# marius311/MuseInference.jl

Hardware: AMD Instinct MI355X
Metric: MC sims/sec (MAP+score) (higher is better)
Workload: dtype f64; 1 GPU; funnel_1e4: Neal's funnel family model=funnel, N=10000-dim z, 1-dim theta, nsims=512 per step (512 on this rank), cold start z0=0, atol=1e-2; element_split=1, parallelism=sims sharded over 1 GPU(s) (weak scaling), one all-gather of scores per step

## Files before the change

museinference.jl_amd/csrc/kernels.hpp:

```cpp
#pragma once
#include <hip/hip_runtime.h>
#include <math.h>
#include <hip/hip_ext.h>
#include <stdint.h>
#include <type_traits>
#include "../../include/muse_hip.h"
#include "solver.hpp"
#include "step.hpp"

namespace muse {



typedef __attribute__((address_space(4))) const uint32_t* kernarg_ptr;
template <bool RAW>
__device__ __forceinline__ void load_problem_theta(const BatchArgs& a, double* args_lds, int p, int tid) {
    if (a.nmaps > 1) {
        wg_barrier<RAW>();
        asm volatile("" : "+v"(tid));
        if (tid < (int)(sizeof(MapTheta) / 4)) {
            uint32_t* dst = reinterpret_cast<uint32_t*>(args_lds) + offsetof(BatchArgs, cur) / 4;
            kernarg_ptr kp = (kernarg_ptr)__builtin_amdgcn_kernarg_segment_ptr();
            dst[tid] = kp[(offsetof(BatchArgs, maps) + (size_t)(p / a.n_per_map) * sizeof(MapTheta)) / 4 + tid];
        }
        wg_barrier<RAW>();
    }
}

template <class P>
struct JacobiPlace : P {};
template <class P>
struct place_is_jacobi : std::false_type {};
template <class P>
struct place_is_jacobi<JacobiPlace<P>> : std::true_type {};

template <class Model, class Place, bool IMPLICIT = false>
__global__ void __launch_bounds__(Place::T) __attribute__((amdgpu_waves_per_eu(Place::kWavesPerEu)))
map_score_kernel(const BatchArgs ) {
    constexpr bool JACOBI = place_is_jacobi<Place>::value;
    static_assert(!JACOBI || (IMPLICIT && !Model::kStencil), "the preconditioned loop is the implicit branch's, for the elementwise models");
    extern __shared__ __attribute__((aligned(16))) unsigned char smem[];
    constexpr int T = Place::T;
    double* red = reinterpret_cast<double*>(smem);
    double* shs = red + 2 * (T / 64) * 8;
    int* ticket = reinterpret_cast<int*>(shs + 40);
    double* args_lds = shs + 42;
    const int tid = threadIdx.x;
#ifdef MUSE_STAMPS
    unsigned long long t_entry;
    asm volatile("s_memtime %0\n\ts_waitcnt lgkmcnt(0)" : "=s"(t_entry)::"memory");
#endif
    {
        kernarg_ptr kp = (kernarg_ptr)__builtin_amdgcn_kernarg_segment_ptr();
        uint32_t* dst = reinterpret_cast<uint32_t*>(args_lds);
        for (int w = tid; w < (int)(kArgsHeadBytes / 4); w += T) dst[w] = kp[w];
        if (tid == 0) ticket[2] = 0;
    }
    __syncthreads();
    const BatchArgs& a = *reinterpret_cast<const BatchArgs*>(args_lds);
    double* exch = args_lds + kArgsDoubles;
    double* lds_x = exch + (Place::kCluster ? kMaxCluster * 8 : 0);
    double* lds_g = lds_x + a.ld + 2;
    const bool wave0 = (__builtin_amdgcn_readfirstlane(tid) >> 6) == 0;
    auto clock_stamp = [&](int k) {
        if (a.clock_out && blockIdx.x == 0 && wave0) {
            unsigned long long t0, t1;
            asm volatile("s_memtime %0\n\ts_memrealtime %1\n\ts_waitcnt lgkmcnt(0)" : "=s"(t0), "=s"(t1)::"memory");
            a.clock_out[2 * k] = t0;
            a.clock_out[2 * k + 1] = t1;
        }
    };
    clock_stamp(0);
    if constexpr (Place::kXgLds) {
        if (tid == 0) {
            lds_x[a.ld] = 0.0;
            lds_g[a.ld] = 0.0;
            lds_x[a.ld + 1] = 0.0;
            lds_g[a.ld + 1] = 0.0;
            if (a.N < a.ld) {
                lds_x[a.N] = 0.0;
                lds_g[a.N] = 0.0;
            }
        }
    }
    if constexpr (Place::kCluster) {
        const int csize = a.csize;
        const int cluster = a.xcd_local ? ((int)(blockIdx.x >> 3) / csize) * 8 + (int)(blockIdx.x & 7) : (int)blockIdx.x / csize;
        const int crank = a.xcd_local ? (int)(blockIdx.x >> 3) % csize : (int)blockIdx.x % csize;
        double* cl_scratch = a.scratch + (int64_t)cluster * a.scratch_stride;
        Solver<Model, Place> sv(a, tid, red, shs);
        sv.crank = crank;
        sv.csize = csize;
        sv.tfirst = crank * T + tid;
        sv.pstride = csize * T;
        sv.pack_blocks();
        sv.cl_part = a.cl_part + (size_t)cluster * kClusterSlotDoubles;
        sv.exch = exch;
        sv.cl_epoch = a.cl_state[cluster];
        int nth = 0;
#ifdef MUSE_STAMPS
        if (tid == 0 && a.stamps && cluster < a.nproblems) a.stamps[(size_t)cluster * 16 + 8] = t_entry;
#endif
        for (int p = cluster; p < a.nproblems; p += a.nclusters, ++nth) {
            sv.bufsel = nth & 1;
            sv.next_p = p + a.nclusters < a.nproblems ? p + a.nclusters : -1;
            sv.parity = 0;
            wg_barrier<!Model::kStencil>();
            load_problem_theta<!Model::kStencil>(a, args_lds, p, tid);
            if constexpr (IMPLICIT && Model::kPair) sv.template run_implicit_pair<JACOBI>(p, cl_scratch, lds_x, lds_g);
            else if constexpr (IMPLICIT) sv.template run_implicit<JACOBI>(p, cl_scratch, lds_x, lds_g);
            else sv.run(p, cl_scratch, lds_x, lds_g);
        }
#ifdef MUSE_STAMPS
        if (cluster < a.nproblems) sv.stamp(cluster + ((a.nproblems - 1 - cluster) / a.nclusters) * a.nclusters, 9);
#endif
        clock_stamp(1);
        if (tid == 0 && crank == 0) {
            a.cl_state[cluster] = sv.cl_epoch;
            if (cluster == 0) a.error_flag[1] = (int)(sv.cl_epoch >> 1);
        }
    } else {
        double* wg_scratch = a.scratch + (int64_t)blockIdx.x * a.scratch_stride;
        unsigned pk0, pk1;
        {
            Solver<Model, Place> s0(a, tid, red, shs);
            s0.pack_blocks();
            pk0 = s0.pk[0];
            pk1 = s0.pk[1];
        }
        int p = (int)blockIdx.x;
        for (;;) {
            int next = 0;
            if (tid == 0) next = atomicAdd(a.work_counter, 1);
#ifdef MUSE_STAMPS
            if (tid == 0 && a.stamps && p < (int)gridDim.x) a.stamps[(size_t)p * 16 + 8] = t_entry;
#endif
            load_problem_theta<!Model::kStencil>(a, args_lds, p, tid);
            {
                Solver<Model, Place> sv(a, tid, red, shs);
                sv.pk[0] = pk0;
                sv.pk[1] = pk1;
                if constexpr (IMPLICIT && Model::kPair) sv.template run_implicit_pair<JACOBI>(p, wg_scratch, lds_x, lds_g);
                else if constexpr (IMPLICIT) sv.template run_implicit<JACOBI>(p, wg_scratch, lds_x, lds_g);
                else sv.run(p, wg_scratch, lds_x, lds_g);
            }
            wg_barrier<!Model::kStencil>();
            if (tid == 0) ticket[0] = next;
            wg_barrier<!Model::kStencil>();
            p = (int)gridDim.x + (__builtin_amdgcn_readfirstlane(ticket[0]) - a.ticket_base);
            if (p >= a.nproblems) break;
        }
        clock_stamp(1);
    }
}

constexpr int kLoopArgsDoubles = (int)((sizeof(LoopArgs) + 7) / 8);
constexpr int kLoopRecDoubles = 7 * kMaxTheta + kMaxTheta * kMaxTheta + 1;
constexpr int kLoopPersistDoubles = kLoopArgsDoubles + kLoopRecDoubles + 3;
enum { STEP_TIMEOUT = 100 };

template <class Place>
struct LoopLds {
    BatchArgs* a;
    double *red, *shs, *lds_x, *lds_g, *persist, *stepbuf, *rec;
    LoopArgs* L;
    int* flags;
    unsigned long long* t_prev;
    __device__ __forceinline__ LoopLds(unsigned char* smem) {
        unsigned z = 0;
        asm volatile("" : "+s"(z));
        red = reinterpret_cast<double*>(smem + z);
        shs = red + 2 * (Place::T / 64) * 8;
        double* args_lds = shs + 42;
        a = reinterpret_cast<BatchArgs*>(args_lds);
        lds_x = args_lds + kArgsDoubles;
        lds_g = lds_x + a->ld + 2;
        persist = Place::kXgLds ? lds_g + a->ld + 2 : lds_x;
        stepbuf = Place::kXgLds ? lds_x : persist + kLoopPersistDoubles;
        L = reinterpret_cast<LoopArgs*>(persist);
        rec = persist + kLoopArgsDoubles;
        flags = reinterpret_cast<int*>(rec + kLoopRecDoubles);
        t_prev = reinterpret_cast<unsigned long long*>(rec + kLoopRecDoubles + 2);
    }
};

#if defined(MUSE_USER_MODEL_HEADER) && defined(MUSE_MODEL_PAIR)
__device__ __forceinline__ void pair_theta_update(int lane, int nt, const int64_t* bnd, const double* th, MapTheta& m) {
    const int K = nt >> 1;
    if (lane < K) {
        double cf[4] = {0.0, 0.0, 0.0, 0.0};
        (void)muse_model_coefs(th[lane], th[K + lane], cf);
        m.t.theta[lane] = th[lane];
        m.t.theta[K + lane] = th[K + lane];
        double* rec = &m.t.sd[0] + 4 * lane;
        rec[0] = cf[0];
        rec[1] = cf[1];
        rec[2] = cf[2];
        rec[3] = cf[3];
    } else if (lane < kMaxTheta / 2) {
        double* rec = &m.t.sd[0] + 4 * lane;
        rec[0] = rec[1] = rec[2] = rec[3] = 0.0;
    }
    if (lane >= 2 * K && lane < kMaxTheta) m.t.theta[lane] = 0.0;
    if (lane == kMaxTheta) {
        double cst = 0.0;
        for (int k = 0; k < K; ++k) {
            double cf[4] = {0.0, 0.0, 0.0, 0.0};
            const double C = muse_model_coefs(th[k], th[K + k], cf);
            cst += (double)(bnd[k + 1] - bnd[k]) * C;
        }
        m.f_const = cst;
        m.pad_ = 0.0;
    }
}
#endif

template <class Model, class Place>
__global__ void __launch_bounds__(Place::T) __attribute__((amdgpu_waves_per_eu(Place::kWavesPerEu)))
muse_loop_kernel(const BatchArgs , const LoopArgs ) {
    static_assert(!Place::kCluster, "one workgroup per element");
    extern __shared__ __attribute__((aligned(16))) unsigned char smem[];
    constexpr int T = Place::T, NW = T / 64;
    const int tid = threadIdx.x;
    {
        kernarg_ptr kp = (kernarg_ptr)__builtin_amdgcn_kernarg_segment_ptr();
        uint32_t* dst = reinterpret_cast<uint32_t*>(reinterpret_cast<double*>(smem) + 2 * (T / 64) * 8 + 42);
        for (int w = tid; w < (int)(kArgsHeadBytes / 4); w += T) dst[w] = kp[w];
    }
    __syncthreads();
    {
        LoopLds<Place> m(smem);
        kernarg_ptr kp = (kernarg_ptr)__builtin_amdgcn_kernarg_segment_ptr();
        uint32_t* dst = reinterpret_cast<uint32_t*>(m.persist);
        for (int w = tid; w < (int)(sizeof(LoopArgs) / 4); w += T) dst[w] = kp[sizeof(BatchArgs) / 4 + w];
        if (tid == 0) {
            unsigned long long now;
            asm volatile("s_memrealtime %0\n\ts_waitcnt lgkmcnt(0)" : "=s"(now)::"memory");
            *m.t_prev = now;
            m.flags[0] = m.flags[1] = m.flags[2] = 0;
        }
    }
    unsigned pk0, pk1;
    {
        LoopLds<Place> m(smem);
        Solver<Model, Place> s0(*m.a, tid, m.red, m.shs);
        s0.pack_blocks();
        pk0 = s0.pk[0];
        pk1 = s0.pk[1];
    }
    const bool solving = ((kernarg_ptr)__builtin_amdgcn_kernarg_segment_ptr())[(sizeof(BatchArgs) + offsetof(LoopArgs, stepper_solves)) / 4] != 0;
    const int stepper_id = (int)gridDim.x - 1;
    const int nworkers = solving ? (int)gridDim.x : (int)gridDim.x - 1;
    const bool stepper = (int)blockIdx.x == stepper_id;
    Prefetch<Place::EPT> pf;
    pf.p = -1;
    pf.have_n1 = pf.have_n2 = pf.have_x = pf.have_xg = pf.g_pending = false;
    typename Place::VZ zkeep;
    zkeep.clear();
    typedef __attribute__((address_space(1))) unsigned long long gu64;
#ifdef MUSE_STAMPS
    auto loop_stamp = [&](int k) {
        LoopLds<Place> m(smem);
        const int b = (int)blockIdx.x, row = b == stepper_id ? 2 : (b == 0 ? 0 : (b == stepper_id / 2 ? 1 : -1));
        if (tid == 0 && m.a->stamps && row >= 0) {
            unsigned long long t;
            asm volatile("s_memrealtime %0\n\ts_waitcnt lgkmcnt(0)" : "=s"(t)::"memory");
            m.a->stamps[(size_t)(m.a->nproblems + row) * 16 + k] = t;
        }
    };
#else
    auto loop_stamp = [](int) {};
#endif
    auto iteration_setup = [&](int it) {
        LoopLds<Place> m(smem);
        BatchArgs& a = *m.a;
        const LoopArgs& L = *m.L;
        a.z0_mode = (it > 1 || L.z0_warm) ? Z0_WARM : Z0_ZERO;
        if (it > 1 && a.ncache) a.ncache_mode = 2;
        a.scores = L.scores_out + (int64_t)(it - 1) * L.scores_stride;
        a.info = L.info_out + (int64_t)(it - 1) * L.info_stride;
        a.gran_tag = L.tag_base + (unsigned)it;
        if constexpr (Place::kXgLds) {
            m.lds_x[a.ld] = 0.0;
            m.lds_g[a.ld] = 0.0;
            m.lds_x[a.ld + 1] = 0.0;
            m.lds_g[a.ld + 1] = 0.0;
            if (a.N < a.ld && pf.p < 0) {
                m.lds_x[a.N] = 0.0;
                m.lds_g[a.N] = 0.0;
            }
        }
    };
    if (!stepper) {
    for (int iter = 1;; ++iter) {
        int err = STEP_OK, converged = 0;
        if (iter == 1 && tid == 0) iteration_setup(1);
        __syncthreads();
        {
            loop_stamp(0);
            {
                LoopLds<Place> m(smem);
                const BatchArgs& a = *m.a;
// ... 603 lines not shown
```

museinference.jl_amd/csrc/muse_engine.cpp:

```cpp
#include <hip/hip_runtime.h>
#include <math.h>
#include <stdint.h>
#include <stdio.h>
#include <stdlib.h>
#include <string.h>

#include <chrono>
#include <string>
#include <thread>
#include <utility>
#include <vector>

#include "../../include/muse_hip.h"
#include "args.hpp"
#include "host_loop.h"
#include "switches.hpp"
#include "user_model.hpp"

using namespace muse;

#if defined(__x86_64__) || defined(__i386__)
#define MUSE_CPU_RELAX() __builtin_ia32_pause()
#elif defined(__aarch64__)
#define MUSE_CPU_RELAX() asm volatile("yield" ::: "memory")
// ... 188 lines not shown
    if (pl == P_R512x10) fixed += (size_t)2 * (c->ld + 2) * sizeof(double);
    return fixed;
}
static int64_t place_scratch_vectors(int pl) {
    return (pl == P_S256 || pl == P_S512) ? 4 + 2 * kM + 1 : pl == P_C256 ? 4 + 2 * kM + 1 + 2 : 2 * kM;
}

static int ensure_zhat(muse_ctx* c, int64_t slots) {
    if (slots <= c->lane->zhat_slots) return MUSE_OK;
    double* nz = nullptr;
    if (hipMalloc(&nz, (size_t)slots * c->ld * sizeof(double)) != hipSuccess)
        return fail(MUSE_ERR_ALLOC, "hipMalloc(zhat) failed");
    HIPCHK(hipMemsetAsync(nz, 0, (size_t)slots * c->ld * sizeof(double), c->lane->stream));
    if (c->lane->zhat) {
        HIPCHK(hipMemcpyAsync(nz, c->lane->zhat, (size_t)c->lane->zhat_slots * c->ld * sizeof(double), hipMemcpyDeviceToDevice,
                              c->lane->stream));
        HIPCHK(hipStreamSynchronize(c->lane->stream));
        HIPCHK(hipFree(c->lane->zhat));
    }
    c->lane->zhat = nz;
    c->lane->zhat_slots = slots;
    return MUSE_OK;
}
static int ensure_scratch(muse_ctx* c, size_t doubles) {
    if (doubles <= c->lane->scratch_doubles) return MUSE_OK;
    HIPCHK(hipStreamSynchronize(c->lane->stream));
    if (c->lane->scratch) HIPCHK(hipFree(c->lane->scratch));
    c->lane->scratch = nullptr;
    c->lane->scratch_doubles = 0;
    if (hipMalloc(&c->lane->scratch, doubles * sizeof(double)) != hipSuccess)
        return fail(MUSE_ERR_ALLOC, "hipMalloc(scratch) failed");
    c->lane->scratch_doubles = doubles;
    return MUSE_OK;
}
static bool ensure_ncache(muse_ctx* c, int64_t slots) {
    if (!ncache_applies(c)) return false;
    if (slots <= c->ncache_slots) return true;
    if (hipStreamSynchronize(c->lane->stream) != hipSuccess) return false;
    if (c->ncache) hipFree(c->ncache);
    c->ncache = nullptr;
    c->ncache_slots = 0;
    c->nc_count = 0;
    if (hipMalloc(&c->ncache, (size_t)slots * 2 * c->ld * sizeof(double)) != hipSuccess) {
        (void)hipGetLastError();
        static bool warned = false;
        if (!warned) {
            fprintf(stderr, "[libmuse_hip] normals cache of %lld slots not allocated: simulations are re-drawn by the generator\n",
                    (long long)slots);
            warned = true;
        }
        return false;
    }
    c->ncache_slots = slots;
    return true;
}
static size_t result_bytes(const muse_ctx* c, int64_t cap) {
    return (size_t)cap * (size_t)c->ntheta * sizeof(double) + (size_t)cap * sizeof(muse_info);
}
static bool ncache_holds(const muse_ctx* c, uint64_t seed, int64_t sim0, int64_t count) {
    return c->ncache && c->nc_count > 0 && c->nc_seed == seed && sim0 >= c->nc_sim0 && sim0 + count <= c->nc_sim0 + c->nc_count;
}
static int ensure_results(muse_ctx* c, int area, int64_t n) {
    if (n <= c->res_cap[area]) return MUSE_OK;
    HIPCHK(hipStreamSynchronize(c->lane->stream));
    if (c->scores_pin[area]) HIPCHK(hipHostFree(c->scores_pin[area]));
    const int64_t cap = n + n / 2 + 16;
    HIPCHK(hipHostMalloc(&c->scores_pin[area], result_bytes(c, cap), hipHostMallocDefault));
    c->info_pin[area] = reinterpret_cast<muse_info*>(c->scores_pin[area] + cap * c->ntheta);
    c->scores_dev[area] = c->scores_pin[area];
    c->info_dev[area] = c->info_pin[area];
    c->res_cap[area] = cap;
    return MUSE_OK;
}

static void common_args(const muse_ctx* c, BatchArgs& a, int64_t stamp_rows) {
    a.N = c->N;
    a.ld = c->ld;
    a.ntheta = c->ntheta;
    for (int k = 0; k <= kMaxTheta; ++k) {
        a.bnd[k] = c->bnd[k];
        a.bnd32[k] = k < nblocks_of(c->ntheta) ? (int)c->bnd[k] : 0x7fffffff;
    }
    a.x_data = c->x_data;
    if (!a.zhat) a.zhat = c->lane->zhat;
    a.work_counter = c->lane->counter;
    if (a.nmaps <= 1) {
        a.nmaps = 1;
        a.n_per_map = a.nproblems;
        a.map_stride = a.nproblems;
    }
    a.debug = c->debug & 0xffff;
    a.stamps = (c->stamps && stamp_rows <= c->stamps_cap) ? c->stamps : nullptr;
    a.csize = 1;
    a.error_flag = c->lane->error_flag;
}
static void attach_ncache(BatchArgs& a, double* cache, int64_t sim0, int64_t count, int mode) {
    a.ncache = cache;
    a.ncache_sim0 = sim0;
    a.ncache_count = (int)count;
    a.ncache_mode = mode;
}

static int launch_batch(muse_ctx* c, BatchArgs& a, hipEvent_t done = nullptr, bool jacobi = false) {
    common_args(c, a, a.nproblems);
    a.clock_out = c->prof_on ? c->clock_pin : nullptr;
    const bool implicit = a.kind == BATCH_IMPLICIT;
    const int pl = implicit ? (use_cluster(c) ? P_C256 : P_S512) : choose_place(c);
    int grid = c->num_cus * place_wgs_per_cu(pl);
    if (place_is_cluster(pl) && c->comm_reserve_cus > 0 && c->num_cus > 2 * c->comm_reserve_cus)
        grid = (c->num_cus - c->comm_reserve_cus) * place_wgs_per_cu(pl);
    if (place_is_cluster(pl) && c->nlanes > 1) grid /= c->nlanes;
    if (place_is_cluster(pl)) {
        const int sharers = c->sw.shared_gpu_ranks;
        if (sharers > 1) grid = grid / sharers > 0 ? grid / sharers : 1;
    }
    a.nclusters = 0;
    if (place_is_cluster(pl)) {
        a.csize = cluster_size(c);
        int ncl = grid / a.csize;
        if (ncl > a.nproblems) ncl = a.nproblems;
        if (ncl < 1) ncl = 1;
        a.nclusters = ncl;
        grid = ncl * a.csize;
        const bool wrap = c->lane->error_flag[1] > 0x30000000;
        if (ncl > c->lane->cl_cap || wrap) {
            HIPCHK(hipStreamSynchronize(c->lane->stream));
            const int cap = ncl > c->lane->cl_cap ? ncl : c->lane->cl_cap;
            if (c->lane->cl_part) HIPCHK(hipFree(c->lane->cl_part));
            if (c->lane->cl_state) HIPCHK(hipFree(c->lane->cl_state));
            c->lane->cl_part = nullptr; c->lane->cl_state = nullptr; c->lane->cl_cap = 0;
            HIPCHK(hipMalloc(&c->lane->cl_part, (size_t)cap * kClusterSlotDoubles * sizeof(double)));
            HIPCHK(hipMalloc(&c->lane->cl_state, (size_t)cap * sizeof(unsigned int)));
            HIPCHK(hipMemsetAsync(c->lane->cl_part, 0, (size_t)cap * kClusterSlotDoubles * sizeof(double), c->lane->stream));
            HIPCHK(hipMemsetAsync(c->lane->cl_state, 0, (size_t)cap * sizeof(unsigned int), c->lane->stream));
            c->lane->error_flag[1] = 0;
            c->lane->cl_cap = cap;
        }
        a.cl_part = c->lane->cl_part;
        a.cl_state = c->lane->cl_state;
        a.xcd_local = (!c->sw.no_xcd_local && ncl % 8 == 0 && !stencil_ctx(c)) ? 1 : 0;
    } else {
        if (grid > a.nproblems) grid = a.nproblems;
        if (grid < 1) grid = 1;
    }
    a.scratch_stride = place_scratch_vectors(pl) * c->ld;
    int rc = ensure_scratch(c, (size_t)(place_is_cluster(pl) ? a.nclusters : grid) * a.scratch_stride);
    if (rc) return rc;
    a.scratch = c->lane->scratch;
    const size_t lds = place_lds(c, pl);
    if (c->lane->ticket_base > 0x70000000u) {
        HIPCHK(hipMemsetAsync(c->lane->counter, 0, 16, c->lane->stream));
        c->lane->ticket_base = 0;
    }
    a.ticket_base = (int)c->lane->ticket_base;
    if (!place_is_cluster(pl)) c->lane->ticket_base += (unsigned)a.nproblems;
    hipEvent_t e0 = c->ev0, e1 = c->ev1;
    if (c->prof_on && (size_t)(2 * c->prof_count + 1) < c->prof_ev.size()) {
        e0 = c->prof_ev[2 * c->prof_count];
        e1 = c->prof_ev[2 * c->prof_count + 1];
        c->prof_count += 1;
    }
    const bool timed = c->timing || c->prof_on;
    if (timed) HIPCHK(hipEventRecord(e0, c->lane->stream));
    {
        LaunchShape shape;
        shape.model = c->model; shape.ntheta = c->ntheta; shape.place = pl; shape.grid = grid; shape.implicit = implicit; shape.lds = lds;
        shape.jacobi = implicit && jacobi;
        shape.big = tier_big(c, pl, a.nmaps);
        shape.lds_s = !implicit && pl == P_C256 && stencil_lds_s(c, a.csize);
        shape.taps = c->stencil_taps;
        shape.noise = c->noise_on;
        shape.link = c->link_on;
        shape.done_event = done;
        const hipError_t e = launch_solver(shape, a, c->lane->stream);
        if (e == hipErrorNotSupported && shape.jacobi)
            rc = fail(MUSE_ERR_INVALID, "this model's preconditioned implicit-differentiation kernel keeps more than 256 bytes of scratch per "
                                        "lane (a header too heavy for its registers): MUSE_IMPLICIT_PL_JACOBI is refused for this library "
                                        "rather than run slower than the loop it replaces -- call without the bit");
        else if (e != hipSuccess) rc = fail(MUSE_ERR_HIP, std::string("solver launch: ") + hipGetErrorString(e));
    }
    if (rc) return rc;
    if (timed) {
        HIPCHK(hipEventRecord(e1, c->lane->stream));
        c->last0 = e0;
        c->last1 = e1;
        c->ev_valid = true;
    }
    return MUSE_OK;
}

static int create_lane(muse_ctx* c, int l) {
    LaneState& ln = c->lanes[l];
    if (ln.ready) return MUSE_OK;
    if (l == 0) ln.stream = c->own_stream;
    else HIPCHK(hipStreamCreateWithFlags(&ln.stream, hipStreamNonBlocking));
    HIPCHK(hipMalloc(&ln.counter, 16));
    HIPCHK(hipMemset(ln.counter, 0, 16));
    HIPCHK(hipHostMalloc(&ln.error_flag, 64, hipHostMallocDefault));
    ln.error_flag[0] = ln.error_flag[1] = 0;
    ln.ready = true;
    return MUSE_OK;
}
static void free_lane(muse_ctx* c, int l) {
    LaneState& ln = c->lanes[l];
    if (!ln.ready) return;
    hipFree(ln.scratch); hipFree(ln.counter); hipFree(ln.cl_part); hipFree(ln.cl_state); hipHostFree(ln.error_flag);
    hipFree(ln.zhat);
    if (l != 0) hipStreamDestroy(ln.stream);
    ln = LaneState();
}
static int use_lane(muse_ctx* c, int l) {
    const int rc = create_lane(c, l);
    if (rc) return rc;
    c->lane = &c->lanes[l];
    return MUSE_OK;
}
template <class F>
static int for_each_lane(muse_ctx* c, F&& f) {
    int rc = MUSE_OK;
    for (int l = 0; l < kMaxLanes && rc == MUSE_OK; ++l)
        if (c->lanes[l].ready) rc = f(c->lanes[l]);
    return rc;
}
static int drain_lanes(muse_ctx* c) {
    return for_each_lane(c, [](LaneState& ln) -> int {
        HIPCHK(hipStreamSynchronize(ln.stream));
        return MUSE_OK;
    });
}

static int settle_area(muse_ctx* c, int area) {
    if (!c->area_inflight[area] || c->nlanes <= 1) return MUSE_OK;
    return drain_lanes(c);
}

#if defined(MUSE_USER_MODEL_HEADER) && defined(MUSE_MODEL_NCONST)
extern "C" {
const double* muse_host_consts[MUSE_MODEL_MAX_CONST] = {nullptr, nullptr, nullptr, nullptr};
long muse_host_const_len[MUSE_MODEL_MAX_CONST] = {0, 0, 0, 0};
}
static muse_ctx* g_consts_owner = nullptr;
static void own_host_constants(muse_ctx* c) {
    if (!c->has_consts || g_consts_owner == c) return;
    for (int k = 0; k < MUSE_MODEL_MAX_CONST; ++k) {
        muse_host_consts[k] = c->consts_host[k];
        muse_host_const_len[k] = c->consts_len[k];
    }
    g_consts_owner = c;
}
#define MUSE_OWN_CONSTANTS(c) own_host_constants(c)
#else
#define MUSE_OWN_CONSTANTS(c) do { } while (0)
#endif
static void set_launch_constants(const muse_ctx* c, BatchArgs& a) {
    for (int k = 0; k < 4; ++k) {
        a.consts[k] = c->consts_dev[k];
        a.const_len[k] = c->consts_len[k];
    }
    if (c->stencil_taps || c->noise_on || c->link_on)
        for (int k = 0; k < kStencilWeights; ++k) a.taps[k] = c->stencil_w[k];
    if (c->noise_on)
        for (int k = 0; k < 2; ++k) a.consts[k] = c->noise_dev[k];
    if (c->link_on) {
        for (int k = 0; k < 2; ++k) a.link[k] = c->link_a[k];
        if (!c->noise_on) a.consts[0] = a.consts[1] = c->link_unit;
    }
}

static int ensure_link_unit(muse_ctx* c, const char* who) {
    if (c->link_unit) return MUSE_OK;
    std::vector<double> ones((size_t)c->ld, 0.0);
    for (int64_t i = 0; i < c->N; ++i) ones[(size_t)i] = 1.0;
    double* fresh = nullptr;
    hipError_t e = hipMalloc(&fresh, (size_t)c->ld * sizeof(double));
    if (e == hipSuccess) e = hipMemcpy(fresh, ones.data(), (size_t)c->ld * sizeof(double), hipMemcpyHostToDevice);
    if (e != hipSuccess) {
        hipFree(fresh);
        return fail(MUSE_ERR_HIP, std::string(who) + ": the unit noise vector: " + hipGetErrorString(e));
    }
    c->link_unit = fresh;
    return MUSE_OK;
}

extern "C" {

const char* muse_last_error(void) { return g_err.c_str(); }
int64_t muse_max_resident_n(void) { return kMaxResidentN; }

const char* muse_model_name(int model) {
#ifdef MUSE_USER_MODEL_HEADER
    return model == MUSE_MODEL_USER ? MUSE_MODEL_NAME : nullptr;
#else
    static const char* const names[3] = {"funnel", "noise", "smooth"};
    return model >= 0 && model <= 2 ? names[model] : nullptr;
#endif
}

int muse_ctx_create(int model, int64_t N, int ntheta, int device, muse_ctx** out) {
    if (!out) return fail(MUSE_ERR_INVALID, "out is NULL");
    *out = nullptr;
    if (model < 0 || model > MUSE_MODEL_USER) return fail(MUSE_ERR_INVALID, "unknown model");
    if (!muse_model_name(model))
        return fail(MUSE_ERR_INVALID, model == MUSE_MODEL_USER
                                          ? "MUSE_MODEL_USER: this library holds the built-in models only (build one from a model "
                                            "header, include/muse_model.h)"
                                          : "this library was built from a user's model header and holds MUSE_MODEL_USER only");
    if (N < 1) return fail(MUSE_ERR_INVALID, "N must be >= 1");
// ... 1631 lines not shown
```

museinference.jl_amd/csrc/solver.hpp:

```cpp
#pragma once
#include <math.h>

#include "models.hpp"
#include "reduce.hpp"
#include "rng.hpp"

namespace muse {

template <int EPT>
struct Prefetch {
    int p;
    bool have_n1;
    bool have_n2;
    bool have_x;
    bool have_xg;
    bool g_pending;
};
#ifndef MUSE_NORMALS_AUX
#define MUSE_NORMALS_AUX 0
#endif
constexpr int kNormalsAux = MUSE_NORMALS_AUX;
typedef __attribute__((address_space(1))) const void* glds_src_t;
typedef __attribute__((address_space(3))) void* glds_dst_t;
template <int T, int EPT>
__device__ __forceinline__ void prefetch_issue(const BatchArgs& a, int tid, int p, double* lds_x, double* lds_g, Prefetch<EPT>& pf,
                                               bool both) {
    const ProblemDesc d = describe(a, p);
    const int64_t ld = a.ld;
    const bool sim = d.x_mode == X_SAMPLE && d.nslot >= 0;
    pf.p = p;
    pf.have_n1 = sim;
    pf.have_n2 = sim && both;
    pf.have_x = d.x_mode == X_DATA && both;
    pf.have_xg = d.x_mode == X_DATA && !both && !(a.debug & 256);
    pf.g_pending = (sim || pf.have_xg) && !both;
    int tl = tid;
    asm volatile("" : "+v"(tl));
    const double* src_x = sim ? a.ncache + (int64_t)(2 * d.nslot + 1) * ld : a.x_data;
    const double* src_g = pf.have_xg ? a.x_data : a.ncache + (int64_t)(2 * d.nslot) * ld;
    const int wave0 = __builtin_amdgcn_readfirstlane(tl) & ~63;
#pragma unroll
    for (int j = 0; j < EPT; ++j) {
        const int i0 = 2 * (tl + j * T);
        if (i0 < (int)ld) {
            const int base = 2 * (wave0 + j * T);
            if (pf.have_n2 || pf.have_x) __builtin_amdgcn_global_load_lds((glds_src_t)(src_x + i0), (glds_dst_t)(lds_x + base), 16, 0, kNormalsAux);
            if (pf.have_n1 || pf.have_xg) __builtin_amdgcn_global_load_lds((glds_src_t)(src_g + i0), (glds_dst_t)(lds_g + base), 16, 0, kNormalsAux);
        }
    }
}

template <bool PAIR>
struct PairState {};
template <>
struct PairState<true> {
    double pc[4], psd[2];
};
template <class Model, class Place>
constexpr bool uniform_linesearch() { return !(Place::kResident && Place::kXgLds && Model::MAXB > 1); }
template <class Model, class Place, bool UNIFORM_LS = uniform_linesearch<Model, Place>()>
struct Solver : PairState<Model::kPair> {
    static constexpr int T = Place::T, EPT = Place::EPT, U = Place::U, MAXB = Model::MAXB;
    static constexpr bool kBig = MAXB > kMaxTheta;
    static constexpr int KB = kBig ? 1 : MAXB;
    static_assert(!kBig || !Place::kResident, "the big tier runs in the streaming placements");
    const double* big_sd;
    const double* big_iv;
    double big_rcpN;
    const BatchArgs& a;
    const int tid;
    double* red;
    double* sh_rho;
    double* sh_gam;
    double* sh_alpha;
    int parity;
    typename Place::VX x;
    typename Place::VG g;
    typename Place::VZ z;
    typename Place::VS s;
    double* hist;
    double iv0, sd0;
    double* sh_sd;
    int f_calls;
    int iter_stamp, stamp_p;
    double last_c, last_gmax;
    int tfirst, pstride;
    __device__ __forceinline__ int ps() const { return Place::kCluster ? pstride : T; }
    int crank, csize;
    unsigned int cl_epoch;
    bool cl_aborted;
    double* cl_part;
    double* exch;

    __device__ Solver(const BatchArgs& a_, int tid_, double* red_, double* shs) : a(a_), tid(tid_), red(red_), parity(0) {
        sh_rho = shs;
        sh_gam = shs + kM;
        sh_alpha = shs + 2 * kM;
        sh_sd = shs + 3 * kM;
        tfirst = tid_;
        pstride = T;
        crank = 0;
        csize = 1;
        cl_epoch = 0;
        cl_aborted = false;
        cl_part = nullptr;
        exch = nullptr;
        gen.p = -1;
        gen.trip = 0;
        gen.active = false;
        bufsel = 0;
        next_p = -1;
    }

    template <int KS, int KM>
    __device__ __forceinline__ void cluster_exchange(double (&sv)[KS > 0 ? KS : 1], double (&mv)[KM > 0 ? KM : 1]) {
        constexpr int K = KS + KM;
        typedef __attribute__((address_space(1))) unsigned long long gu64;
        cl_epoch += 1;
        gu64* gran = (gu64*)cl_part + (size_t)(cl_epoch & 1u) * (kMaxCluster * 16);
        if (tid < 64) {
            int lane = tid;
            asm volatile("" : "+v"(lane));
            if (lane < 2 * K) {
                double v = 0.0;
#pragma unroll
                for (int k = 0; k < K; ++k) {
                    const double vk = k < KS ? sv[k < KS ? k : 0] : mv[k >= KS ? k - KS : 0];
                    v = (lane >> 1) == k ? vk : v;
                }
                const unsigned long long b = (unsigned long long)__double_as_longlong(v);
                const unsigned half = (lane & 1) ? (unsigned)(b >> 32) : (unsigned)(b & 0xffffffffull);
                __hip_atomic_store(gran + crank * 16 + lane, ((unsigned long long)cl_epoch << 32) | half, __ATOMIC_RELAXED,
                                   __HIP_MEMORY_SCOPE_AGENT);
            }
            constexpr bool kLiveOnly = Model::kStencil;
            const int total = kLiveOnly ? csize * 2 * K : csize * 16;
            unsigned spins = 0;
            unsigned long long t_wait0 = 0;
            for (int q0 = 0; q0 < total; q0 += 64) {
                const int ql = q0 + lane;
                const int q = kLiveOnly ? (ql / (2 * K)) * 16 + ql % (2 * K) : ql;
                const bool live = ql < total && (kLiveOnly || (q & 15) < 2 * K);
                unsigned long long gv = 0;
                for (;;) {
                    bool ok = true;
                    if (live) {
                        gv = __hip_atomic_load(gran + q, __ATOMIC_RELAXED, __HIP_MEMORY_SCOPE_AGENT);
                        ok = (unsigned)(gv >> 32) == cl_epoch;
                    }
                    if (__builtin_amdgcn_ballot_w64(!ok) == 0ull || cl_aborted) break;
                    if ((++spins & 0x3ffu) == 0) {
                        unsigned long long now;
                        asm volatile("s_memrealtime %0\n\ts_waitcnt lgkmcnt(0)" : "=s"(now)::"memory");
                        if (t_wait0 == 0) t_wait0 = now;
                        else if (now - t_wait0 > 400000000ull) {
                            __hip_atomic_store((gi32*)a.error_flag, 1, __ATOMIC_RELAXED, __HIP_MEMORY_SCOPE_SYSTEM);
                            cl_aborted = true;
                        }
                    }
                }
                if (live) reinterpret_cast<unsigned*>(exch)[q] = (unsigned)(gv & 0xffffffffull);
            }
        }
        wg_barrier<!Model::kStencil>();
#pragma unroll
        for (int k = 0; k < K; ++k) {
            double acc = exch[k];
            for (int c = 1; c < csize; ++c) {
                const double v = exch[c * 8 + k];
                acc = k < KS ? acc + v : __builtin_fmax(acc, v);
            }
            if (k < KS) sv[k < KS ? k : 0] = uniform(acc);
            else mv[k >= KS ? k - KS : 0] = uniform(acc);
        }
    }
    template <int KS, int KM>
    __device__ __forceinline__ void reduce(double (&sv)[KS > 0 ? KS : 1], double (&mv)[KM > 0 ? KM : 1]) {
        if constexpr (Place::kCluster && Model::kStencil) asm volatile("s_waitcnt vmcnt(0)" ::: "memory");
        block_allreduce<T, KS, KM, !Model::kStencil>(sv, mv, red, parity, tid);
        if constexpr (Place::kCluster) cluster_exchange<KS, KM>(sv, mv);
    }
    __device__ __forceinline__ void pass_barrier() {
        if constexpr (Place::kCluster) {
            asm volatile("s_waitcnt vmcnt(0)" ::: "memory");
            __syncthreads();
            double z1[1] = {0.0}, z2[1] = {0.0};
            cluster_exchange<1, 0>(z1, z2);
        } else {
            __syncthreads();
        }
    }
    __device__ __forceinline__ void stamp(int p, int k) const {
#ifdef MUSE_STAMPS
        if (tid == 0 && a.stamps) {
            unsigned long long t;
            asm volatile("s_memtime %0\n\ts_waitcnt lgkmcnt(0)" : "=s"(t)::"memory");
            a.stamps[(size_t)p * 16 + k] = t;
        }
#else
        (void)p; (void)k;
#endif
    }
    using VH = typename Place::VH;
    __device__ __forceinline__ VH hdx(int slot) const {
        VH v;
        v.bind(hist + (int64_t)(2 * slot) * a.ld, a.ld);
        return v;
    }
    __device__ __forceinline__ VH hdg(int slot) const {
        VH v;
        v.bind(hist + (int64_t)(2 * slot + 1) * a.ld, a.ld);
        return v;
    }
    unsigned pk[2];
    __device__ __forceinline__ int blk(int jj, int i) const {
        if constexpr (MAXB == 1) return 0;
        else if constexpr (kBig) return block_of_big((int)a.N, a.ntheta, big_rcpN, i);
        else if constexpr (Place::kResident) {
            unsigned w = pk[jj / 10];
            asm volatile("" : "+v"(w));
            return (int)((w >> (3 * (jj % 10))) & 7u);
        }
        else return block_of<MAXB>(a, i);
    }
    __device__ __forceinline__ double ivk(int jj, int i) const {
        if constexpr (MAXB == 1) return iv0;
        else if constexpr (kBig) return big_iv[blk(jj, i)];
        else return a.cur.t.iv[blk(jj, i)];
    }
    __device__ __forceinline__ double sdk(int jj, int i) const {
        if constexpr (MAXB == 1) return sd0;
        else if constexpr (kBig) return big_sd[blk(jj, i)];
        else return sh_sd[blk(jj, i)];
    }
    __device__ __forceinline__ double sdk_at(int i) const {
        if constexpr (MAXB == 1) return sd0;
        else if constexpr (kBig) return big_sd[blk(0, i)];
        else return sh_sd[block_of<MAXB>(a, i)];
    }
    __device__ __forceinline__ auto gcoef(int jj, int i) const {
        if constexpr (Model::kPair && MAXB == 2) {
            const bool valid = i < (int)a.N;
            PairGv c;
#pragma unroll
            for (int q = 0; q < 4; ++q) c.c[q] = valid ? this->pc[q] : 0.0;
            return c;
        } else if constexpr (Model::kPair) {
            PairGp c;
            c.p = pair_table(a.cur.t) + 4 * blk(jj, i);
            c.valid = i < (int)a.N;
            return c;
        } else {
            return ivk(jj, i);
        }
    }
    __device__ __forceinline__ auto scoef_of_block(int k) const {
        PairS c;
        if constexpr (MAXB == 2) {
            c.c[0] = this->psd[0];
            c.c[1] = this->psd[1];
        } else {
            c.c[0] = sh_sd[2 * k];
            c.c[1] = sh_sd[2 * k + 1];
        }
// ... 1120 lines not shown
                            double xo[2], so[2];
                            gen_pair(i0, xo, so);
                            store_f64x2(x.rsrc, i0, xo[0], xo[1]);
                            store_f64x2(s.rsrc, i0, so[0], so[1]);
                        }
                        double sum[4] = {gen.sum[0], gen.sum[1], gen.sum[2], gen.sum[3]}, mx[2] = {gen.mx[0], gen.mx[1]};
                        reduce<4, 2>(sum, mx);
                        init_f = 0.5 * (sum[0] + a.cur.f_const);
                        init_dphi = sum[1];
                        init_gmax = nan_if(sum[0] != sum[0] || sum[1] != sum[1], mx[0]);
                        trial_c = 1.0;
                        trial_phi = 0.5 * (sum[2] + a.cur.f_const);
                        trial_dphi = sum[3];
                        trial_gmax = nan_if(sum[2] != sum[2] || sum[3] != sum[3], mx[1]);
                        init_done = true;
                        z_zero = true;
                    }
                }
                if constexpr (!Model::kStencil) {
                    if (!init_done && z_from_sample && !d.normals_only) {
                        const bool ztrue_start = d.z0_mode == Z0_TRUE;
                        double sum[4] = {0.0, 0.0, 0.0, 0.0}, mx[2] = {0.0, 0.0};
                        constexpr int kGenU = Place::kResident ? 1 : kStreamGenU;
                        NormalPair npv[2 * kGenU];
                        for_elems_pre<T, EPT, kGenU>(ld, tfirst, ps(), [&](auto ucount, int i0, int pstr) {
                            constexpr int UU = decltype(ucount)::value;
                            uint64_t idx[2 * UU];
                            NormalPair got[2 * UU];
#pragma unroll
                            for (int u = 0; u < UU; ++u) {
                                idx[2 * u] = (uint64_t)(i0 + 2 * u * pstr);
                                idx[2 * u + 1] = (uint64_t)(i0 + 2 * u * pstr + 1);
                            }
                            normal_pairs<2 * UU>(a.seed, sim, idx, got);
#pragma unroll
                            for (int q = 0; q < 2 * UU; ++q) npv[q] = got[q];
                        }, [&](int jj, int i) {
                            const bool valid = i < N;
                            const NormalPair np = npv[jj % (2 * kGenU)];
                            double zt, xt;
                            Model::sample(scoef(jj, i), np.n1, np.n2, zt, xt, i);
                            zt = valid ? zt : 0.0;
                            xt = valid ? xt : 0.0;
                            if constexpr (KEEP_ZTRUE) ztrue.set(jj, i, keep_value(valid, zt, sdk(jj, i), np, i));
                            x.set(jj, i, xt);
                            const double z0v = ztrue_start ? zt : 0.0;
                            if (Place::kResident || ztrue_start) z.set(jj, i, z0v);
                            const auto ivi = gcoef(jj, i);
                            const double gi = Model::grad(ivi, xt, z0v, sum[0], i);
                            const double sd = -gi;
                            s.set(jj, i, sd);
                            sum[1] = fma(gi, sd, sum[1]);
                            mx[0] = absmax(mx[0], gi);
                            const double zt1 = fma(1.0, sd, z0v);
                            const double gt = Model::grad(ivi, xt, zt1, sum[2], i);
                            sum[3] = fma(gt, sd, sum[3]);
                            mx[1] = absmax(mx[1], gt);
                        }, when(KEEP_ZTRUE, ztrue), x, s, when(Place::kResident || ztrue_start, z));
                        reduce<4, 2>(sum, mx);
                        init_f = 0.5 * (sum[0] + a.cur.f_const);
                        init_dphi = sum[1];
                        init_gmax = nan_if(sum[0] != sum[0] || sum[1] != sum[1], mx[0]);
                        trial_c = 1.0;
                        trial_phi = 0.5 * (sum[2] + a.cur.f_const);
                        trial_dphi = sum[3];
                        trial_gmax = nan_if(sum[2] != sum[2] || sum[3] != sum[3], mx[1]);
                        init_done = true;
                        z_zero = !ztrue_start && !Place::kResident;
                    }
                }
                if (!init_done)
                for_elems<T, EPT, US>(ld, tfirst, ps(), [&](int jj, int i) {
                    const bool valid = i < N;
                    const NormalPair np = normal_pair(a.seed, sim, (uint64_t)i);
                    double zt, xt;
                    if constexpr (Model::kStencil) {
                        zt = sdk(jj, i) * np.n1;
                        xt = np.n2;
                        g.set(jj, i, valid ? zt : 0.0);
                    } else {
                        Model::sample(scoef(jj, i), np.n1, np.n2, zt, xt, i);
                    }
                    zt = valid ? zt : 0.0;
                    xt = valid ? xt : 0.0;
                    if constexpr (KEEP_ZTRUE) ztrue.set(jj, i, keep_value(valid, zt, sdk(jj, i), np, i));
                    x.set(jj, i, xt);
                    if (d.z0_mode == Z0_ZERO) z.set(jj, i, 0.0);
                    else if (d.z0_mode == Z0_TRUE) z.set(jj, i, zt);
                    else if constexpr (Place::kResident) z.set(jj, i, z0src.get(jj, i));
                }, when(Model::kStencil, g), when(KEEP_ZTRUE, ztrue), x, when(z_from_sample, z));
                if constexpr (!Place::kResident) {
                    if (!init_done && !z_from_sample && !z_in_place)
                        for_elems<T, EPT, U>(ld, tfirst, ps(), [&](int jj, int i) { z.set(jj, i, z0src.get(jj, i)); }, z);
                }
            }
            if constexpr (Model::kStencil) {
                pass_barrier();
                const NoiseVec<Model, 1> sn;
                for_elems<T, EPT, U>(ld, tfirst, ps(), [&](int jj, int i) {
                    const bool valid = i < N;
                    const int ic = valid ? i : 0;
                    const int im = ic == 0 ? (int)N - 1 : ic - 1, ip = ic == (int)N - 1 ? 0 : ic + 1;
                    const double zl = g.get1(im), zr = g.get1(ip);
                    const double az = stencil_apply<Model>(zl, g.get1(ic), zr);
                    if constexpr (link_model<Model>()) {
                        const double si = sn.get(jj, i);
                        const double xv = fma(si, x.get(jj, i), link_value<Model>(az));
                        x.set(jj, i, valid && si != 0.0 ? xv : 0.0);
                    } else
                    if constexpr (noise_model<Model>()) {
                        const double si = sn.get(jj, i);
                        const double xv = fma(si, x.get(jj, i), az);
                        x.set(jj, i, valid && si != 0.0 ? xv : 0.0);
                    } else {
                        const double xv = az + x.get(jj, i);
                        x.set(jj, i, valid ? xv : 0.0);
                    }
                }, x);
            }
        } else {
            VH xs;
            xs.bind(d.x_mode == X_DATA ? a.x_data : a.x_given, ld);
            x.clear(); g.clear(); z.clear(); s.clear();
            const bool z_zero = d.z0_mode == Z0_ZERO || d.z0_mode == Z0_TRUE;
            bool done = false;
            if constexpr (Place::kResident && Place::kXgLds) {
                if (pf_hit && pf.have_x && d.x_mode == X_DATA && !z_zero) {
                    asm volatile("s_waitcnt vmcnt(0)" ::: "memory");
                    for_elems<T, EPT, U>(ld, tfirst, ps(), [&](int jj, int i) { z.set(jj, i, z0src.get(jj, i)); });
                    done = true;
                } else if (pf_hit && pf.have_xg && d.x_mode == X_DATA && !z_zero) {
                    asm volatile("s_waitcnt vmcnt(0)" ::: "memory");
                    for_elems<T, EPT, U>(ld, tfirst, ps(), [&](int jj, int i) {
                        x.set(jj, i, g.get(jj, i));
                        z.set(jj, i, z0src.get(jj, i));
                    });
                    done = true;
                }
            }
            if (!done)
            for_elems<T, EPT, U>(ld, tfirst, ps(), [&](int jj, int i) {
                x.set(jj, i, xs.get(jj, i));
                if (z_zero) z.set(jj, i, 0.0);
                else if (!z_in_place) z.set(jj, i, z0src.get(jj, i));
            }, x, when(z_zero || !z_in_place, z));
        }
        if (pf_hit) {
            if constexpr (Place::kResident && Place::kXgLds) {
                if (pf.g_pending) asm volatile("s_waitcnt vmcnt(0)" ::: "memory");
            }
            pf.p = -1;
            pf.g_pending = false;
        }
        stamp(p, 9);
        if constexpr (Model::kStencil) pass_barrier();
        else wg_barrier<true>();
        if constexpr (kBg && !KEEP_ZTRUE) {
            gen.active = false;
            const bool same_map = a.nmaps <= 1 || next_p / a.n_per_map == p / a.n_per_map;
            if (next_p >= 0 && d.tsample < 0 && same_map) {
                const ProblemDesc dn = describe(a, next_p);
                if (dn.x_mode == X_SAMPLE && dn.z0_mode == Z0_ZERO && !dn.normals_only && dn.tsample < 0) {
                    gen.p = next_p;
                    gen.trip = 0;
                    gen.sim = (uint64_t)dn.sim;
#pragma unroll
                    for (int k = 0; k < 4; ++k) gen.sum[k] = 0.0;
                    gen.mx[0] = gen.mx[1] = 0.0;
                    gen.active = true;
                    double* xb = bufsel ? wg_scratch : wg_scratch + (int64_t)(4 + 2 * kM + 1) * ld;
                    double* sb = bufsel ? wg_scratch + 2 * ld : xb + ld;
                    bg_xr = make_rsrc(xb, ld * 8);
                    bg_sr = make_rsrc(sb, ld * 8);
                }
            }
        }

        stamp(p, 1);
    }

    static constexpr bool kPrefetchTwoLoop = !Place::kResident && Place::kCluster && Model::kStencil;
    template <class F>
    __device__ __forceinline__ void pass_ab(VH& A, VH& B, F&& f) {
        int t = tfirst;
        asm volatile("" : "+v"(t));
        const int n = (int)a.ld, pstr = pstride;
#pragma unroll 1
        for (int i0 = 2 * t; i0 < n; i0 += 2 * U * pstr) {
#pragma unroll
            for (int u = 0; u < U; ++u) {
                const int i = i0 + 2 * u * pstr;
                f(2 * u, i);
                f(2 * u + 1, i + 1);
            }
            s.template flush<U>(i0, pstr);
            A.unload();
            B.unload();
        }
    }
    __device__ __forceinline__ double twoloop_prefetched(int upper, int lower, double dot0) {
        if constexpr (kPrefetchTwoLoop) {
            double dot = dot0;
            int t0 = tfirst;
            asm volatile("" : "+v"(t0));
            auto fetch = [&](VH& v) { v.template preload<U>(2 * t0, pstride); };
            VH A = hdg((upper - 1) % kM), B = A;
            if (upper > lower) B = hdx((upper - 2) % kM);
            for (int index = upper; index >= lower; --index) {
                const int slot = (index - 1) % kM;
                const double al = sh_rho[slot] * dot;
                if ((tid & 63) == 0) sh_alpha[slot] = al;
                double sum[1] = {0.0}, mx[1] = {0.0};
                if (index > lower) {
                    pass_ab(A, B, [&](int jj, int i) {
                        const double qi = fma(-al, A.get(jj, i), s.get(jj, i));
                        s.set(jj, i, qi);
                        sum[0] = fma(B.get(jj, i), qi, sum[0]);
                    });
                } else {
                    const double gam = sh_gam[(upper - 1) % kM];
                    pass_ab(A, B, [&](int jj, int i) {
                        const double dgi = A.get(jj, i);
                        const double si = gam * fma(-al, dgi, s.get(jj, i));
                        s.set(jj, i, si);
                        sum[0] = fma(dgi, si, sum[0]);
                    });
                }
                if (index > lower) {
                    A = hdg((index - 2) % kM);
                    fetch(A);
                    if (index - 1 > lower) {
                        B = hdx((index - 3) % kM);
                        fetch(B);
                    }
                } else {
                    A = hdx((lower - 1) % kM);
                    fetch(A);
                    if (lower < upper) {
                        B = hdg(lower % kM);
                        fetch(B);
                    } else {
                        fetch(g);
                    }
                }
                reduce<1, 0>(sum, mx);
                dot = sum[0];
            }
            for (int index = lower; index <= upper; ++index) {
                const int slot = (index - 1) % kM;
                const double beta = sh_rho[slot] * dot;
                const double coef = sh_alpha[slot] - beta;
                double sum[1] = {0.0}, mx[1] = {0.0};
                if (index < upper) {
                    pass_ab(A, B, [&](int jj, int i) {
                        const double si = fma(A.get(jj, i), coef, s.get(jj, i));
                        s.set(jj, i, si);
                        sum[0] = fma(B.get(jj, i), si, sum[0]);
                    });
                    A = hdx(index % kM);
                    fetch(A);
                    if (index + 1 < upper) {
                        B = hdg((index + 1) % kM);
                        fetch(B);
                    } else {
                        fetch(g);
                    }
                } else {
                    pass_ab(A, g, [&](int jj, int i) {
                        const double si = -fma(A.get(jj, i), coef, s.get(jj, i));
                        s.set(jj, i, si);
                        sum[0] = fma(g.get(jj, i), si, sum[0]);
                    });
                }
                reduce<1, 0>(sum, mx);
                dot = sum[0];
            }
            return dot;
        } else {
            (void)upper; (void)lower;
            return dot0;
        }
    }

    __device__ __forceinline__ void solve(int p) {
        const int64_t ld = a.ld;
        const int N = (int)a.N;
        f_calls = 0;
        iter_stamp = 99;
        stamp_p = p;
        last_c = NAN;
        constexpr bool kFuseInit = Place::kResident && !Model::kStencil;
        double dphi_init;
        bool init_fused = kFuseInit;
        if (init_done) {
            f = init_f;
            dphi_init = init_dphi;
            gmax = init_gmax;
            f_calls = 1;
            have_trial = true;
            init_fused = true;
        } else if constexpr (kFuseInit) {
            eval_init_with_trial(1.0, f, dphi_init, gmax);
        } else {
            have_trial = false;
            eval<false, true, Model::kStencil>(0.0, f, dphi_init, gmax);
            if constexpr (Model::kStencil) init_fused = true;
// ... 825 lines not shown
```

Measured before the change: 12.34 million sims/s.

## Hand off work-stealing ticket inside solver barrier and double-buffer ticket slot

The persistent work-stealing loop no longer uses two extra workgroup barriers after each problem to publish the next ticket. Thread 0 now writes the ticket into an alternating LDS slot just before a barrier that already exists inside the solver. The grid offset is folded into ticket_base on the host. Per-map theta loading now goes through scalar kernarg loads written as 16-byte chunks, the atomic uses agent scope with relaxed ordering, and stamps-only timing instrumentation is added; in exchange the loop relies on the solver always reaching that barrier.

```diff
diff --git a/museinference.jl_amd/csrc/kernels.hpp b/museinference.jl_amd/csrc/kernels.hpp
--- a/museinference.jl_amd/csrc/kernels.hpp
+++ b/museinference.jl_amd/csrc/kernels.hpp
@@ -18,10 +18,17 @@
     if (a.nmaps > 1) {
         wg_barrier<RAW>();
         asm volatile("" : "+v"(tid));
-        if (tid < (int)(sizeof(MapTheta) / 4)) {
-            uint32_t* dst = reinterpret_cast<uint32_t*>(args_lds) + offsetof(BatchArgs, cur) / 4;
-            kernarg_ptr kp = (kernarg_ptr)__builtin_amdgcn_kernarg_segment_ptr();
-            dst[tid] = kp[(offsetof(BatchArgs, maps) + (size_t)(p / a.n_per_map) * sizeof(MapTheta)) / 4 + tid];
+        uint2* dst = reinterpret_cast<uint2*>(reinterpret_cast<unsigned char*>(args_lds) + offsetof(BatchArgs, cur));
+        const int m = p / __builtin_amdgcn_readfirstlane(a.n_per_map);
+        kernarg_ptr kp = (kernarg_ptr)__builtin_amdgcn_kernarg_segment_ptr() + (offsetof(BatchArgs, maps) + (size_t)m * sizeof(MapTheta)) / 4;
+#pragma unroll 1
+        for (int j = 0; j < (int)(sizeof(MapTheta) / 16); ++j) {
+            uint32_t v0 = kp[4 * j], v1 = kp[4 * j + 1], v2 = kp[4 * j + 2], v3 = kp[4 * j + 3];
+            asm volatile("" : "+s"(v0), "+s"(v1), "+s"(v2), "+s"(v3));
+            if (tid == j) {
+                dst[2 * j] = make_uint2(v0, v1);
+                dst[2 * j + 1] = make_uint2(v2, v3);
+            }
         }
         wg_barrier<RAW>();
     }
@@ -56,7 +63,14 @@
         for (int w = tid; w < (int)(kArgsHeadBytes / 4); w += T) dst[w] = kp[w];
         if (tid == 0) ticket[2] = 0;
     }
+#ifdef MUSE_STAMPS
+    unsigned long long t_fetch, t_bar;
+    asm volatile("s_waitcnt vmcnt(0)\n\ts_memtime %0\n\ts_waitcnt lgkmcnt(0)" : "=s"(t_fetch)::"memory");
+#endif
     __syncthreads();
+#ifdef MUSE_STAMPS
+    asm volatile("s_memtime %0\n\ts_waitcnt lgkmcnt(0)" : "=s"(t_bar)::"memory");
+#endif
     const BatchArgs& a = *reinterpret_cast<const BatchArgs*>(args_lds);
     double* exch = args_lds + kArgsDoubles;
     double* lds_x = exch + (Place::kCluster ? kMaxCluster * 8 : 0);
@@ -66,8 +80,10 @@
         if (a.clock_out && blockIdx.x == 0 && wave0) {
             unsigned long long t0, t1;
             asm volatile("s_memtime %0\n\ts_memrealtime %1\n\ts_waitcnt lgkmcnt(0)" : "=s"(t0), "=s"(t1)::"memory");
-            a.clock_out[2 * k] = t0;
-            a.clock_out[2 * k + 1] = t1;
+            typedef __attribute__((address_space(1))) unsigned long long gu64;
+            gu64* co = (gu64*)a.clock_out;
+            co[2 * k] = t0;
+            co[2 * k + 1] = t1;
         }
     };
     clock_stamp(0);
@@ -129,25 +145,35 @@
             pk1 = s0.pk[1];
         }
         int p = (int)blockIdx.x;
+        int slot = 0;
         for (;;) {
             int next = 0;
-            if (tid == 0) next = atomicAdd(a.work_counter, 1);
+            if (tid == 0) {
+                gi32* wc = (gi32*)a.work_counter;
+                asm volatile("" : "+v"(wc));
+                next = __hip_atomic_fetch_add(wc, 1, __ATOMIC_RELAXED, __HIP_MEMORY_SCOPE_AGENT);
+            }
 #ifdef MUSE_STAMPS
-            if (tid == 0 && a.stamps && p < (int)gridDim.x) a.stamps[(size_t)p * 16 + 8] = t_entry;
+            if (tid == 0 && a.stamps && p < (int)gridDim.x) {
+                const unsigned long long df = (t_fetch - t_entry) >> 4, db = (t_bar - t_entry) >> 4;
+                a.stamps[(size_t)p * 16 + 8] = (1ull << 63) | ((db < 1023 ? db : 1023) << 53) | ((df < 1023 ? df : 1023) << 43) |
+                                               (t_entry & ((1ull << 43) - 1));
+            }
 #endif
             load_problem_theta<!Model::kStencil>(a, args_lds, p, tid);
             {
                 Solver<Model, Place> sv(a, tid, red, shs);
                 sv.pk[0] = pk0;
                 sv.pk[1] = pk1;
+                sv.tk_slot = ticket + slot;
+                sv.tk_next = next;
                 if constexpr (IMPLICIT && Model::kPair) sv.template run_implicit_pair<JACOBI>(p, wg_scratch, lds_x, lds_g);
                 else if constexpr (IMPLICIT) sv.template run_implicit<JACOBI>(p, wg_scratch, lds_x, lds_g);
                 else sv.run(p, wg_scratch, lds_x, lds_g);
             }
-            wg_barrier<!Model::kStencil>();
-            if (tid == 0) ticket[0] = next;
-            wg_barrier<!Model::kStencil>();
-            p = (int)gridDim.x + (__builtin_amdgcn_readfirstlane(ticket[0]) - a.ticket_base);
+            if constexpr (Model::kStencil) __syncthreads();
+            p = __builtin_amdgcn_readfirstlane(ticket[slot]) - a.ticket_base;
+            slot ^= 1;
             if (p >= a.nproblems) break;
         }
         clock_stamp(1);
diff --git a/museinference.jl_amd/csrc/muse_engine.cpp b/museinference.jl_amd/csrc/muse_engine.cpp
--- a/museinference.jl_amd/csrc/muse_engine.cpp
+++ b/museinference.jl_amd/csrc/muse_engine.cpp
@@ -364,7 +364,7 @@
         HIPCHK(hipMemsetAsync(c->lane->counter, 0, 16, c->lane->stream));
         c->lane->ticket_base = 0;
     }
-    a.ticket_base = (int)c->lane->ticket_base;
+    a.ticket_base = (int)c->lane->ticket_base - (place_is_cluster(pl) ? 0 : grid);
     if (!place_is_cluster(pl)) c->lane->ticket_base += (unsigned)a.nproblems;
     hipEvent_t e0 = c->ev0, e1 = c->ev1;
     if (c->prof_on && (size_t)(2 * c->prof_count + 1) < c->prof_ev.size()) {
diff --git a/museinference.jl_amd/csrc/solver.hpp b/museinference.jl_amd/csrc/solver.hpp
--- a/museinference.jl_amd/csrc/solver.hpp
+++ b/museinference.jl_amd/csrc/solver.hpp
@@ -110,6 +110,17 @@
         gen.active = false;
         bufsel = 0;
         next_p = -1;
+        tk_slot = nullptr;
+        tk_next = 0;
+    }
+    int* tk_slot;
+    int tk_next;
+    __device__ __forceinline__ void hand_ticket() {
+        if (tk_slot != nullptr) {
+            int v = tk_next;
+            asm volatile("" : "+v"(v));
+            if (tid == 0) *tk_slot = v;
+        }
     }
 
     template <int KS, int KM>
@@ -1536,6 +1547,7 @@
             pf.p = -1;
             pf.g_pending = false;
         }
+        hand_ticket();
         stamp(p, 9);
         if constexpr (Model::kStencil) pass_barrier();
         else wg_barrier<true>();
```

After: 12.42 million sims/s, median of 6. Within noise of the previous version (+0.6%).
